# JuanLuisGonzalez/FAL_net

Hardware: AMD Instinct MI355X
Metric: stereo-pairs/sec Stage-1 step @256x512 N=49 (higher is better)
Workload: dtype bf16; 1 GPU; Stage-1 training step (BASELINE configs[1]), batch 8/GPU, 256x512, N=49, seeded weights, seeded VGG19; global_batch=8, parallelism=dp1, launch=eager launches, recorded sequences issued by falnet_replay (C)

## Files before the change

### fal_net_amd/_lib.py

```python
import ctypes as C
import os
import threading

import torch

F32, BF16, F16 = 0, 1, 2
ACT_NONE, ACT_ELU, ACT_RELU = 0, 1, 2
OUT_NHWC, OUT_PLANAR_F32 = 0, 1
CPAD = 32

DETERMINISTIC = os.environ.get("FALNET_DETERMINISTIC") == "1"

def ab(name, default):
    if os.environ.get("FALNET_AB") != "1":
        return default
    return os.environ.get(name, default)


_LIB_PATH = os.environ.get("FALNET_LIB") or os.path.join(os.path.dirname(os.path.abspath(__file__)), "libfalnet_hip.so")


class Src(C.Structure):
    _fields_ = [("ptr", C.c_void_p), ("C", C.c_int32), ("H", C.c_int32), ("W", C.c_int32),
                ("sb", C.c_int64), ("sy", C.c_int64), ("sx", C.c_int64)]
# ... 57 lines not shown
_P, _I, _L, _F, _D = C.c_void_p, C.c_int, C.c_int64, C.c_float, C.c_double
SIGNATURES = {
    "falnet_version": [],
    "falnet_last_error": [],
    "falnet_channel_pad": [_I],
    "falnet_set_device": [_I],
    "falnet_set_deterministic": [_I],
    "falnet_get_deterministic": [],
    "falnet_conv2d": [C.POINTER(Conv), _P],
    "falnet_conv3x3_c3": [_P, _P, _P, _P, _I, _I, _I, _I, _I, _I, _P],
    "falnet_conv2d_multi": [C.POINTER(Conv), _I, _P],
    "falnet_conv2d_kernel_name": [C.POINTER(Conv), C.c_char_p, _I],
    "falnet_wgrad_workspace_bytes": [C.POINTER(Wgrad)],
    "falnet_wgrad": [C.POINTER(Wgrad), _P],
    "falnet_wgrad_fuses_bias": [C.POINTER(Wgrad)],
    "falnet_wgrad_reduce": [_P, _I, _I, _I, _I, _P, _I, _I, _I, _I, _I, _P],
    "falnet_bias_grad": [_P, _L, _I, _I, _P, _I, _I, _P],
    "falnet_pack_weights_batched": [_P, _I, _I, _I, _P],
    "falnet_adam_pack_batched": [_P, _I, _I, _I, _L, _L, _L, _P, _F, _F, _F, _F, _P, _P],
    "falnet_adam_ranges": [_P, _L, _L, _L, _P, _I, _P, _F, _F, _F, _F, _P, _P],
    "falnet_adam_tick": [_P, _P, _P],
    "falnet_pack_up2_batched": [_P, _I, _I, _I, _P],
    "falnet_wgrad_reduce_batched": [_P, _I, _I, _I, _P],
    "falnet_wgrad_reduce_blocks": [_I, _I, _I],
    "falnet_bias_grad_batched": [_P, _I, _I, _I, _P],
    "falnet_bias_grad_batched_det": [_P, _I, _I, _I, _P, _L, _P],
    "falnet_pack_weights": [_P, _I, _I, _I, _I, _I, _I, _I, _P, _P, _I, _P],
    "falnet_nchw_to_nhwc": [_P, _P, _I, _I, _I, _I, _I, _I, _P],
    "falnet_nhwc_to_nchw": [_P, _P, _I, _I, _I, _I, _I, _I, _P],
    "falnet_upsample_bwd": [_P, _P, _P, _I, _I, _I, _I, _I, _I, _I, _P],
# ... 305 lines not shown
```

### fal_net_amd/csrc/conv.hip

```cpp
#include <limits.h>
#include <stdlib.h>
#include <type_traits>
#include "common.h"
#include "conv_epilogue.h"

#define CONV_THREADS 256
#define CONV_BM 128
#define ROWB 64
#define ROWP 80

template <typename T> struct KC;
template <> struct KC<float> { static constexpr int value = 16; };
template <> struct KC<bf16_t> { static constexpr int value = 32; };
template <> struct KC<f16_t> { static constexpr int value = 32; };

template <typename T> struct Vec8 {
    uint4 v;
    __device__ __forceinline__ void load(const T* p) { v = *reinterpret_cast<const uint4*>(p); }
    __device__ __forceinline__ void store(T* p) const { *reinterpret_cast<uint4*>(p) = v; }
    __device__ __forceinline__ float get(int i) const {
        const unsigned w = (&v.x)[i >> 1];
        return (i & 1) ? H16<T>::hi(w) : H16<T>::lo(w);
    }
    __device__ __forceinline__ void set8(const float (&f)[8]) {
// ... 3058 lines not shown
        const dim3 eg((unsigned)((total + 255) / 256 > 1024 ? 1024 : (total + 255) / 256), (unsigned)n);
#define SPLITK_M(T) hipLaunchKernelGGL(splitk_epilogue_multi_kernel<T>, eg, dim3(256), 0, st, pp)
        FALNET_DISPATCH_DTYPE(descs[0].dtype, SPLITK_M);
#undef SPLITK_M
    }
    FALNET_RETURN_LAUNCH();
}

static inline int round32(int v) { return (v + 31) / 32 * 32; }

extern "C" int64_t falnet_wgrad_workspace_bytes(const falnet_wgrad_t* p) {
    if (!p) return -1;
    return (int64_t)p->nsplit * p->ntaps * round32(p->gC) * p->cin_total * (int64_t)sizeof(float);
}

enum WgradKernel { WGK_BAD = -1, WGK_TAP = 0, WGK_PATCH11, WGK_PATCH12, WGK_PATCH21, WGK_S2, WGK_C3, WGK_ROWS, WGK_ROWS_S2, WGK_WAVE };
bool falnet_wgrad_rows_applicable(const falnet_wgrad_t& p);
int falnet_wgrad_rows_launch(const falnet_wgrad_t& p, hipStream_t st);
bool falnet_wgrad_rows_s2_applicable(const falnet_wgrad_t& p);
int falnet_wgrad_rows_s2_launch(const falnet_wgrad_t& p, hipStream_t st);
bool falnet_wgrad_wave_applicable(const falnet_wgrad_t& p);
int falnet_wgrad_wave_launch(const falnet_wgrad_t& p, hipStream_t st);
bool falnet_wgrad_c3wave_applicable(const falnet_wgrad_t& p);
int falnet_wgrad_c3wave_launch(const falnet_wgrad_t& p, hipStream_t st);

static bool canonical_taps9(const falnet_wgrad_t& p) {
    if (p.ntaps != 9) return false;
    for (int t = 0; t < 9; ++t)
        if (p.tap_dy[t] != t / 3 - 1 || p.tap_dx[t] != t % 3 - 1) return false;
    return true;
}

static WgradKernel choose_wgrad_kernel(const falnet_wgrad_t& p) {
    const int w_rows = round32(p.gC);
    const bool h16 = p.dtype == FALNET_BF16 || p.dtype == FALNET_F16;
    const bool canon = canonical_taps9(p);
    if (p.up2 && p.variant != 7) { falnet_set_error("wgrad: up2 (a deconv layer's gradient on the low-resolution grid) is a mode of variant 7 only"); return WGK_BAD; }
    if (p.variant == 6) {
        const bool ok = h16 && canon && p.isy == 1 && p.isx == 1 && p.TH == p.IH && p.TW == p.IW && p.gC == 32 && w_rows == 32 && p.cin_total == 32 && p.nsrc == 1;
// ... 4 lines not shown
        bool ok = h16 && canon && p.isy == 2 && p.isx == 2 && p.TW >= 16 && p.TH == (p.IH + 1) / 2 && p.TW == (p.IW + 1) / 2;
        for (int s = 0; s < p.nsrc && ok; ++s) ok = p.src[s].C % 32 == 0 && ((p.src[s].H == p.IH && p.src[s].W == p.IW) || (p.src[s].sy == 0 && p.src[s].sx == 0));
        if (!ok) { falnet_set_error("wgrad: variant 5 needs a 16-bit 3x3 stride-2 pad-1 launch with sources at the input size"); return WGK_BAD; }
        return WGK_S2;
    }
    if (p.variant == 8) {
        if (!falnet_wgrad_rows_s2_applicable(p)) { falnet_set_error("wgrad: variant 8 needs a 16-bit 3x3 stride-2 pad-1 launch with ONE source at the input size"); return WGK_BAD; }
        return WGK_ROWS_S2;
    }
    if (p.variant == 9) {
        if (!falnet_wgrad_wave_applicable(p)) { falnet_set_error("wgrad: variant 9 needs a 16-bit dense 3x3 stride-1 launch over ONE 32-channel NHWC source at the launch size, gC 32 or 64, TW >= 32"); return WGK_BAD; }
        return WGK_WAVE;
    }
    if (p.variant == 7) {
        if (!falnet_wgrad_rows_applicable(p)) { falnet_set_error("wgrad: variant 7 needs a 16-bit dense 3x3 stride-1 launch with sources at the launch size or half of it (up2: ONE source at the launch size, nsplit a multiple of 4)"); return WGK_BAD; }
        return WGK_ROWS;
    }
    const bool dense = canon && p.isy == 1 && p.isx == 1 && p.TH == p.IH && p.TW == p.IW && p.TW >= 16 && !g_disable_patch && p.variant != 1;
    if (dense) {
        if (p.variant == 3 || p.variant == 4) {
            const bool co2 = p.variant == 3;
            if (!(h16 && (co2 ? w_rows : p.cin_total) % 64 == 0)) { falnet_set_error("wgrad: variant %d needs 16-bit operands and a channel count that is a multiple of 64", p.variant); return WGK_BAD; }
            return co2 ? WGK_PATCH12 : WGK_PATCH21;
        }
        return WGK_PATCH11;
    }
    return WGK_TAP;
}

static int check_wgrad_desc(const falnet_wgrad_t& p) {
    FALNET_CHECK_ARG(p.dtype == FALNET_F32 || p.dtype == FALNET_BF16 || p.dtype == FALNET_F16, "wgrad: bad dtype %d", p.dtype);
// ... 4 lines not shown
            if (int r = check_src(p.src[s], 32, "wgrad")) return r;
            ctot += p.src[s].C;
        }
        FALNET_CHECK_ARG(ctot == p.cin_total, "wgrad: sources carry %d channels, cin_total=%d", ctot, p.cin_total);
    } else {
        FALNET_CHECK_ARG(p.src[0].ptr && p.src[0].C == 3, "wgrad: variant 6 needs a 3-channel planar f32 source");
    }
    FALNET_CHECK_ARG(p.gout && p.gC > 0 && p.gC % 32 == 0 && p.nsplit >= 1 && p.ntaps >= 1 && p.ntaps <= 9, "wgrad: bad argument");
    FALNET_CHECK_ARG(p.B > 0 && p.TH > 0 && p.TW > 0, "wgrad: empty shape");
    FALNET_CHECK_ARG(p.cout >= 0 && p.cout <= p.gC, "wgrad: cout=%d exceeds gC=%d", p.cout, p.gC);
    return 0;
}

static bool wgrad_kernel_fuses_bias(WgradKernel k) {
    if (falnet_deterministic()) return false;
    return k == WGK_PATCH11 || k == WGK_PATCH12 || k == WGK_PATCH21 || k == WGK_S2 || k == WGK_C3 || k == WGK_ROWS || k == WGK_ROWS_S2 || k == WGK_WAVE;
}

extern "C" int falnet_wgrad_fuses_bias(const falnet_wgrad_t* pp) {
    if (!pp || check_wgrad_desc(*pp) != 0) return 0;
    return wgrad_kernel_fuses_bias(choose_wgrad_kernel(*pp)) ? 1 : 0;
}

extern "C" int falnet_wgrad(const falnet_wgrad_t* pp, void* stream) {
    FALNET_ENTER(stream);
    FALNET_CHECK_ARG(pp, "wgrad: null descriptor");
    falnet_wgrad_t p = *pp;
    if (int r = check_wgrad_desc(p)) return r;
    FALNET_CHECK_ARG(p.partial, "wgrad: no workspace");
    if (p.cout == 0) p.cout = p.gC;
    const int w_rows = round32(p.gC);
    const WgradKernel k = choose_wgrad_kernel(p);
    if (k == WGK_BAD) return -1;
    if (p.bias_grad && !wgrad_kernel_fuses_bias(k)) {
        falnet_set_error("wgrad: bias_grad is set but the selected kernel (%d) cannot fuse it -- ask falnet_wgrad_fuses_bias first", (int)k);
        return -3;
    }
    hipStream_t st = (hipStream_t)stream;
    const int tiles_x = (p.TW + WP_TW - 1) / WP_TW, tiles_y = (p.TH + WP_TH - 1) / WP_TH;
    const int npatch = p.B * tiles_x * tiles_y;
    const int pps = (npatch + p.nsplit - 1) / p.nsplit;
    switch (k) {
    case WGK_ROWS:
        return falnet_wgrad_rows_launch(p, st);
    case WGK_ROWS_S2:
        return falnet_wgrad_rows_s2_launch(p, st);
    case WGK_WAVE:
        return falnet_wgrad_wave_launch(p, st);
    case WGK_C3:
        if (falnet_wgrad_c3wave_applicable(p)) return falnet_wgrad_c3wave_launch(p, st);
#define WG_C3(T) hipLaunchKernelGGL(HIP_KERNEL_NAME(wgrad3x3_c3_kernel<T>), dim3(1, 1, p.nsplit), dim3(WC3_THREADS), 0, st, p, w_rows, tiles_x, tiles_y, pps)
        FALNET_DISPATCH_16(p.dtype, WG_C3);
        break;
    case WGK_S2:
#define WG_S2_2(T) hipLaunchKernelGGL(HIP_KERNEL_NAME(wgrad3x3_s2_kernel<T, 2>), dim3(p.cin_total / 32, w_rows / 64, p.nsplit), dim3(WP_THREADS), 0, st, p, w_rows, tiles_x, tiles_y, pps)
#define WG_S2_1(T) hipLaunchKernelGGL(HIP_KERNEL_NAME(wgrad3x3_s2_kernel<T, 1>), dim3(p.cin_total / 32, w_rows / 32, p.nsplit), dim3(WP_THREADS), 0, st, p, w_rows, tiles_x, tiles_y, pps)
        if (w_rows % 64 == 0) FALNET_DISPATCH_16(p.dtype, WG_S2_2);
        else FALNET_DISPATCH_16(p.dtype, WG_S2_1);
        break;
// ... 76 lines not shown
```

### fal_net_amd/csrc/wgrad_rows.hip

```cpp
#include <stdlib.h>
#include "common.h"

typedef float f32x16 __attribute__((ext_vector_type(16)));
typedef __bf16 bf16x8 __attribute__((ext_vector_type(8)));
typedef _Float16 f16x8 __attribute__((ext_vector_type(8)));
typedef short s16x4 __attribute__((ext_vector_type(4)));
typedef short s16x8 __attribute__((ext_vector_type(8)));

template <typename T> struct Mma16;
template <> struct Mma16<bf16_t> {
    static __device__ __forceinline__ f32x16 mma(s16x8 a, s16x8 b, f32x16 c) {
        return __builtin_amdgcn_mfma_f32_32x32x16_bf16(__builtin_bit_cast(bf16x8, a), __builtin_bit_cast(bf16x8, b), c, 0, 0, 0);
    }
    static __device__ __forceinline__ float f32(short v) { return __uint_as_float(((unsigned)(unsigned short)v) << 16); }
};
template <> struct Mma16<f16_t> {
    static __device__ __forceinline__ f32x16 mma(s16x8 a, s16x8 b, f32x16 c) {
        return __builtin_amdgcn_mfma_f32_32x32x16_f16(__builtin_bit_cast(f16x8, a), __builtin_bit_cast(f16x8, b), c, 0, 0, 0);
    }
    static __device__ __forceinline__ float f32(short v) { return (float)__builtin_bit_cast(_Float16, v); }
};

#define WR_THREADS 256
#define WR_TW 32
// ... 1200 lines not shown
            float* dst = p.partial + (((int64_t)split * 9 + dy * 3 + dx) * w_rows) * p.cin_total;
#pragma unroll
            for (int j4 = 0; j4 < 4; ++j4) {
                const float4 o = *reinterpret_cast<const float4*>(red + ((dy * 3 + dx) * 4 + j4) * 256);
                const float v[4] = {acc[dy][dx][4 * j4] + o.x, acc[dy][dx][4 * j4 + 1] + o.y, acc[dy][dx][4 * j4 + 2] + o.z, acc[dy][dx][4 * j4 + 3] + o.w};
#pragma unroll
                for (int e = 0; e < 4; ++e) {
                    const int j = 4 * j4 + e;
                    const int co = co0 + 32 * c_t + (j & 3) + 8 * (j >> 2) + 4 * h;
                    if (ci < p.cin_total && co < w_rows) dst[(int64_t)co * p.cin_total + ci] = v[e];
                }
            }
        }
}

bool falnet_wgrad_rows_s2_applicable(const falnet_wgrad_t& p) {
    if (p.dtype != FALNET_BF16 && p.dtype != FALNET_F16) return false;
    if (p.ntaps != 9 || p.isy != 2 || p.isx != 2 || p.TH != (p.IH + 1) / 2 || p.TW != (p.IW + 1) / 2) return false;
    for (int t = 0; t < 9; ++t)
        if (p.tap_dy[t] != t / 3 - 1 || p.tap_dx[t] != t % 3 - 1) return false;
    if (p.gC % 32 || p.cin_total % 32 || p.nsrc != 1) return false;
    const falnet_src_t& S = p.src[0];
    if (S.C != p.cin_total || S.H != p.IH || S.W != p.IW || S.sx == 0 || S.sy == 0) return false;
    if ((int64_t)p.B * ((p.TW + WR_TW - 1) / WR_TW) * p.TH >= (1ll << 30)) return false;
    return true;
}

int falnet_wgrad_rows_s2_launch(const falnet_wgrad_t& p, hipStream_t st) {
    const int w_rows = (p.gC + 31) / 32 * 32;
    const int ntci = (p.cin_total + 63) / 64, ntco = (w_rows + 63) / 64;
// ... 68 lines not shown
    if (form == 84) {
        if (p.dtype == FALNET_F16) hipLaunchKernelGGL(HIP_KERNEL_NAME(wgrad3x3_rows8_kernel<f16_t, 4, 0, true, true, 4>), grid, dim3(WR8_THREADS), 0, st, p, w_rows, ntci, ntiles, nstrips);
        else hipLaunchKernelGGL(HIP_KERNEL_NAME(wgrad3x3_rows8_kernel<bf16_t, 4, 0, true, true, 4>), grid, dim3(WR8_THREADS), 0, st, p, w_rows, ntci, ntiles, nstrips);
        FALNET_RETURN_LAUNCH();
    }
#endif
    if (p.up2) {
        if (p.dtype == FALNET_F16) hipLaunchKernelGGL(HIP_KERNEL_NAME(wgrad3x3_rows16_kernel<f16_t, 4, 2, true>), grid, dim3(WR8_THREADS), 0, st, p, w_rows, ntci, ntiles, nstrips);
        else hipLaunchKernelGGL(HIP_KERNEL_NAME(wgrad3x3_rows16_kernel<bf16_t, 4, 2, true>), grid, dim3(WR8_THREADS), 0, st, p, w_rows, ntci, ntiles, nstrips);
        FALNET_RETURN_LAUNCH();
    }
    if (p.dtype == FALNET_F16) hipLaunchKernelGGL(HIP_KERNEL_NAME(wgrad3x3_rows16_kernel<f16_t, 4, 2, false>), grid, dim3(WR8_THREADS), 0, st, p, w_rows, ntci, ntiles, nstrips);
    else hipLaunchKernelGGL(HIP_KERNEL_NAME(wgrad3x3_rows16_kernel<bf16_t, 4, 2, false>), grid, dim3(WR8_THREADS), 0, st, p, w_rows, ntci, ntiles, nstrips);
    FALNET_RETURN_LAUNCH();
}
```

### fal_net_amd/ops.py

```python
import ctypes as C
import os
import sys

import torch

from . import _lib as L

CPAD = L.CPAD
H16 = (torch.bfloat16, torch.float16)
TYPE_SYM = {torch.bfloat16: "DF16b", torch.float16: "DF16_", torch.float32: "f"}

TIMER = None
AUTOTUNE = os.environ.get("FALNET_AUTOTUNE", "1") != "0"
DETERMINISTIC = L.DETERMINISTIC
UP2W = L.ab("FALNET_UP2W", "0") == "1"
UP2D = L.ab("FALNET_UP2D", "1") == "1"


_PKG_CACHE = os.path.join(os.path.dirname(os.path.abspath(__file__)), "autotune_cache.json")
_CACHE_PATH = os.environ.get("FALNET_AUTOTUNE_CACHE", _PKG_CACHE)
_CACHE_WRITABLE = ("FALNET_AUTOTUNE_CACHE" in os.environ and _CACHE_PATH != "0") or os.environ.get("FALNET_AUTOTUNE_CACHE_WRITE") == "1"
_GATES = {"FALNET_NO_DMA": "0", "FALNET_WS2": "1", "FALNET_S2F_DMA": "1", "FALNET_S2D_DMA": "1", "FALNET_S2_SPLITK": "1",
          "FALNET_GATHER_NARROW": "0", "FALNET_S2_MULTI": None, "FALNET_SMALL_TILE_DMA": "1", "FALNET_UP2": "1", "FALNET_DEEP": "1", "FALNET_TILE8": "1"}
if os.environ.get("FALNET_AB") == "1" and any(os.environ.get(k, v) != v for k, v in _GATES.items()):
# ... 509 lines not shown
                lib.falnet_conv2d(ref, st)
            e1.record()
            e1.synchronize()
            tt = e0.elapsed_time(e1)
            t = tt if t is None else min(t, tt)
        if _AUTOTUNE_LOG:
            print(f"[autotune] M={M} w_rows={w_rows} Cout={Cout} ntaps={d.ntaps} nsrc={d.nsrc} v{v} k{k}: {t / reps * 1e3:.1f} us", file=sys.stderr)
        if best_t is None or t < best_t:
            best, best_t = (v, k), t
    return best


def _wgrad_plan(dtype, srcs, taps, stride_in, B, TH, TW, IH, IW, cin_pad, cout_pad, max_slabs, target_wgs=1536, up2=False):
    M = B * TH * TW
    h16 = dtype in (torch.bfloat16, torch.float16)
    tn = TYPE_SYM[dtype]
    dense = len(taps) == 9 and stride_in == 1 and TW >= 16
    c3 = len(srcs) == 1 and srcs[0].C == 3
    npatch = B * ((TH + 3) // 4) * ((TW + 31) // 32)
    if c3:
        assert h16 and dense and cout_pad == 32 and cin_pad == 32, "variant 6: 16-bit first layer, Cout 32"
        variant, nsplit, sym = 6, max(1, min(_WGRAD_WGS, npatch)), f"_Z18wgrad3x3_c3_kernelI{tn}Ev14falnet_wgrad_tiiii"
        if IW % 4 == 0 and TW >= 32 and not DETERMINISTIC:
            nsplit = max(1, min(_WGRAD_WAVE_WGS, B * ((TW + 31) // 32) * TH // (8 * _WGRAD_WAVE_MIN_ROWS)))
            sym = f"_Z22wgrad3x3_c3wave_kernelI{tn}Ev14falnet_wgrad_ti"
    elif _wgrad_s2(dtype, taps, stride_in, TH, TW, IH, IW, srcs) and _wgrad_wave_s2(srcs, IH, IW, TW, cin_pad, cout_pad):
        units = B * ((TW + 31) // 32) * TH
        nsplit = max(1, min(_WGRAD_WAVE_WGS, units // _WGRAD_WAVE_MIN_ROWS))
        variant, sym = 9, f"_Z22wgrad3x3_wave32_kernelI{tn}Li2ELb1EEv14falnet_wgrad_ti"
    elif _wgrad_s2(dtype, taps, stride_in, TH, TW, IH, IW, srcs) and _wgrad_rows_s2(srcs, IH, IW, TW, cin_pad, cout_pad):
        tiles = ((cin_pad + 63) // 64) * ((cout_pad + 63) // 64)
        units = B * ((TW + 31) // 32) * TH
        nsplit = max(1, min(_WGRAD_ROWS_WGS // tiles, units // _WGRAD_ROWS_MIN_ROWS))
        if nsplit >= 8:
            nsplit -= nsplit % 8
        variant, sym = 8, f"_Z23wgrad3x3_rows8s2_kernelI{tn}Li2EEv14falnet_wgrad_tiiii"
    elif _wgrad_s2(dtype, taps, stride_in, TH, TW, IH, IW, srcs):
        tiles = (cin_pad // 32) * (cout_pad // (64 if cout_pad % 64 == 0 else 32))
        variant, nsplit = 5, max(1, min((_WGRAD_WGS + tiles - 1) // tiles, npatch))
        sym = f"_Z18wgrad3x3_s2_kernelI{tn}Li{2 if cout_pad % 64 == 0 else 1}EEv14falnet_wgrad_tiiii"
    elif _wgrad_wave(dtype, dense, srcs, IH, IW, TW, cin_pad, cout_pad) and not up2:
        npw = 8 // (cout_pad // 32)
        units = B * ((TW + 31) // 32) * TH
        nsplit = max(1, min(_WGRAD_WAVE_WGS, units // (npw * _WGRAD_WAVE_MIN_ROWS)))
        variant, sym = 9, f"_Z22wgrad3x3_wave32_kernelI{tn}Li{cout_pad // 32}ELb0EEv14falnet_wgrad_ti"
    elif _wgrad_rows(dtype, dense, srcs, IH, IW, TW, cin_pad, cout_pad):
        tiles = ((cin_pad + 63) // 64) * ((cout_pad + 63) // 64)
        units = B * ((TW + 31) // 32) * TH * (4 if up2 else 1)
        nsplit = max(1, min(_WGRAD_ROWS_WGS // tiles, units // _WGRAD_ROWS_MIN_ROWS))
        if nsplit >= 8:
            nsplit -= nsplit % 8
        if up2:
            nsplit = max(4, nsplit - nsplit % 4)
            max_slabs -= max_slabs % 4
            if max_slabs < 4:
                raise ValueError("up2 weight gradient: the slab budget holds fewer than four slabs")
        variant, sym = 7, f"_Z22wgrad3x3_rows16_kernelI{tn}Li4ELi2ELb{int(up2)}EEv14falnet_wgrad_tiiii"
    elif up2:
        raise ValueError("up2 weight gradient: the row-streaming kernel does not apply")
    elif dense:
        co2 = _wgrad_co2(dtype, dense, cin_pad, cout_pad)
        tiles = (cin_pad // 32) * (cout_pad // 32) // (2 if co2 else 1)
        nsplit = max(1, min((_WGRAD_WGS + tiles - 1) // tiles, npatch))
        variant = 3 if co2 else 0
        sym = f"_Z21wgrad3x3_patch_kernelI{tn}Li1ELi{2 if co2 else 1}EEv14falnet_wgrad_tiiii"
    else:
        tiles = ((cin_pad + 63) // 64) * ((cout_pad + 63) // 64) * len(taps)
        variant, nsplit, sym = 0, max(1, min((target_wgs + tiles - 1) // tiles, (M + 255) // 256)), f"_Z12wgrad_kernelI{tn}Ev14falnet_wgrad_ti"
    return variant, max(1, min(nsplit, max_slabs)), sym


def _fill_wgrad(d, dtype, srcs, IH, IW, gout, taps, stride_in, B, TH, TW, pc):
    d.nsrc = len(srcs)
    for i, s in enumerate(srcs):
        d.src[i] = s
    d.IH, d.IW = IH, IW
    gC = gout.shape[-1]
    d.gout, d.gC, d.cout = gout.data_ptr(), gC, pc.cout
    _fill_taps(d, taps)
    d.isy = d.isx = stride_in
    d.B, d.TH, d.TW = B, TH, TW
    d.cin_total = pc.cin_pad
    d.dtype = L.dtype_code(dtype)

# ... 4 lines not shown
    if lib.falnet_wgrad_fuses_bias(C.byref(d)) != 1:
        return False
    d.bias_grad = grad_b.data_ptr()
    return True



def wgrad_calls(dtype, srcs, IH, IW, gout, taps, stride_in, B, TH, TW, pc, grad_w, grad_b, ws, target_wgs=1536,
                name="wgrad", flops=0, up2=False):
    lib = L.lib()
    d = L.Wgrad()
    _fill_wgrad(d, dtype, srcs, IH, IW, gout, taps, stride_in, B, TH, TW, pc)
    gC = gout.shape[-1]
    M = B * TH * TW * (4 if up2 else 1)
    slab = len(taps) * pad_c(gC) * pc.cin_pad * 4
    d.variant, nsplit, sym = _wgrad_plan(dtype, srcs, taps, stride_in, B, TH, TW, IH, IW, pc.cin_pad, pad_c(gC), ws.numel() * 4 // slab,
                                         target_wgs, up2=up2)
    d.nsplit = nsplit
    d.up2 = int(up2)
    d.partial = ws.data_ptr()
    assert lib.falnet_wgrad_workspace_bytes(C.byref(d)) <= ws.numel() * 4, "wgrad workspace too small"
    ref = C.byref(d)
    c0_real, c0_pad = pc.group_channels()
    npix = M
    keep = (d, srcs, gout, grad_w, grad_b, ws)

    def k_wgrad(accumulate=0, _keep=keep):
        L.check(lib.falnet_wgrad(ref, L.stream_ptr()), name)

    fused_bias = _fuse_bias(lib, d, grad_b)

    def k_reduce(accumulate=0):
        st = L.stream_ptr()
        L.check(lib.falnet_wgrad_reduce(L.ptr(ws), d.nsplit, len(taps), pad_c(gC), pc.cin_pad, L.ptr(grad_w), pc.cout, pc.cin, c0_real, c0_pad,
# ... 72 lines not shown
    SLAB_CAP = int(L.ab("FALNET_SLAB_CAP_MB", "32")) << 20

    def __init__(self, dtype, device):
        self.dtype, self.device = dtype, device
        self.items, self.bias = [], []
        self.ws = None
        self.accumulate = 1

    def add(self, srcs, IH, IW, gout, taps, stride_in, B, TH, TW, pc, grad_w, grad_b, name="wgrad", flops=0, bucket=0, up2=False):
        lib = L.lib()
        d = L.Wgrad()
        _fill_wgrad(d, self.dtype, srcs, IH, IW, gout, taps, stride_in, B, TH, TW, pc)
        gC = gout.shape[-1]
        M = B * TH * TW * (4 if up2 else 1)
        slab = len(taps) * pad_c(gC) * pc.cin_pad * 4
        d.variant, nsplit, sym = _wgrad_plan(self.dtype, srcs, taps, stride_in, B, TH, TW, IH, IW, pc.cin_pad, pad_c(gC), max(1, self.SLAB_CAP // slab),
                                             up2=up2)
        d.nsplit = nsplit
        d.up2 = int(up2)
        ref = C.byref(d)
        keep = (d, srcs, gout, grad_w, grad_b)

        post = []

        def launch(_keep=keep):
            L.check(lib.falnet_wgrad(ref, L.stream_ptr()), name)
        c0_real, c0_pad = pc.group_channels()
        self.items.append(dict(bucket=bucket, post=post, d=d, bytes=nsplit * slab, nsplit=nsplit, ntaps=len(taps), w_rows=pad_c(gC), cin_total=pc.cin_pad,
                               cout=pc.cout, cin=pc.cin, c0_real=c0_real, c0_pad=c0_pad, grad=grad_w))
        if not _fuse_bias(lib, d, grad_b) and grad_b is not None:
            self.bias.append(dict(bucket=bucket, g=gout, npix=M, gC=gC, cout=pc.cout, db=grad_b))
        t_launch = _timed(sym, flops, 0, launch, name)

        def launch_and_reduce():
# ... 111 lines not shown
```

### include/falnet_hip.h

```cpp
#ifndef FALNET_HIP_H
#define FALNET_HIP_H

#include <stdint.h>

#ifdef __cplusplus
extern "C" {
#endif

enum { FALNET_F32 = 0, FALNET_BF16 = 1, FALNET_F16 = 2 };
enum { FALNET_ACT_NONE = 0, FALNET_ACT_ELU = 1, FALNET_ACT_RELU = 2 };
enum { FALNET_OUT_NHWC = 0, FALNET_OUT_PLANAR_F32 = 1 };

int falnet_version(void);
const char* falnet_last_error(void);
int falnet_channel_pad(int dtype);
int falnet_set_device(int device);
int falnet_set_deterministic(int on);
int falnet_get_deterministic(void);

typedef struct {
    const void* ptr;
    int32_t C;
    int32_t H, W;
    int64_t sb, sy, sx;
// ... 49 lines not shown
    int32_t gC;
    int32_t ntaps;
    int32_t tap_dy[9], tap_dx[9];
    int32_t isy, isx;
    int32_t B, TH, TW;
    int32_t cin_total;
    int32_t nsplit;
    float* partial;
    int32_t dtype;
    int32_t variant;
    float* bias_grad;
    int32_t cout;
    int32_t up2;
} falnet_wgrad_t;
int falnet_wgrad_fuses_bias(const falnet_wgrad_t* p);
int64_t falnet_wgrad_workspace_bytes(const falnet_wgrad_t* p);
int falnet_wgrad(const falnet_wgrad_t* p, void* stream);
int falnet_wgrad_reduce(const float* partial, int nsplit, int ntaps, int cout_pad, int cin_total,
                        float* grad, int cout, int cin, int c0_real, int c0_pad, int accumulate, void* stream);
int falnet_bias_grad(const void* g, int64_t npix, int gC, int cout, float* db,
                     int accumulate, int dtype, void* stream);

int falnet_wgrad_reduce_blocks(int cout, int cin_total, int groups);
typedef struct {
    const float* partial; float* grad;
    int32_t nsplit, ntaps, w_rows, cin_total, cout, cin, c0_real, c0_pad, groups, block_begin;
} falnet_reduce_t;
typedef struct {
    const void* g; float* db; int64_t npix;
    int32_t gC, cout, blocks, block_begin;
// ... 135 lines not shown
```

Before: 1530 stereo-pairs/s.

## Add rows32 wgrad kernel processing two row pairs per step for non-up2 variant 7

Adds a new weight-gradient kernel for the row-streaming 3x3 stride-1 path. It consumes two output rows per pipeline step with a double-size LDS ring slot, and splits the row range between two wave groups that reduce their results through LDS at the end. The aim is fewer barriers per row and more MFMA reuse of loaded gradient and input rows. It becomes the default for non-up2 variant 7, with an env override back to rows16. Kernel-name reporting moves from Python into a C API so profiling symbols match the new dispatch. The cost is higher LDS and register use, which may reduce occupancy.

```diff
diff --git a/fal_net_amd/_lib.py b/fal_net_amd/_lib.py
--- a/fal_net_amd/_lib.py
+++ b/fal_net_amd/_lib.py
@@ -95,6 +95,7 @@
     "falnet_wgrad_workspace_bytes": [C.POINTER(Wgrad)],
     "falnet_wgrad": [C.POINTER(Wgrad), _P],
     "falnet_wgrad_fuses_bias": [C.POINTER(Wgrad)],
+    "falnet_wgrad_kernel_name": [C.POINTER(Wgrad), C.c_char_p, _I],
     "falnet_wgrad_reduce": [_P, _I, _I, _I, _I, _P, _I, _I, _I, _I, _I, _P],
     "falnet_bias_grad": [_P, _L, _I, _I, _P, _I, _I, _P],
     "falnet_pack_weights_batched": [_P, _I, _I, _I, _P],
diff --git a/fal_net_amd/csrc/conv.hip b/fal_net_amd/csrc/conv.hip
--- a/fal_net_amd/csrc/conv.hip
+++ b/fal_net_amd/csrc/conv.hip
@@ -3096,15 +3096,21 @@
     return (int64_t)p->nsplit * p->ntaps * round32(p->gC) * p->cin_total * (int64_t)sizeof(float);
 }
 
-enum WgradKernel { WGK_BAD = -1, WGK_TAP = 0, WGK_PATCH11, WGK_PATCH12, WGK_PATCH21, WGK_S2, WGK_C3, WGK_ROWS, WGK_ROWS_S2, WGK_WAVE };
+enum WgradKernel { WGK_BAD = -1, WGK_TAP = 0, WGK_PATCH11, WGK_PATCH12, WGK_PATCH21, WGK_S2, WGK_C3, WGK_ROWS, WGK_ROWS_S2, WGK_WAVE, WGK_ROWS32 };
 bool falnet_wgrad_rows_applicable(const falnet_wgrad_t& p);
 int falnet_wgrad_rows_launch(const falnet_wgrad_t& p, hipStream_t st);
+int falnet_wgrad_rows32_launch(const falnet_wgrad_t& p, hipStream_t st);
 bool falnet_wgrad_rows_s2_applicable(const falnet_wgrad_t& p);
 int falnet_wgrad_rows_s2_launch(const falnet_wgrad_t& p, hipStream_t st);
 bool falnet_wgrad_wave_applicable(const falnet_wgrad_t& p);
 int falnet_wgrad_wave_launch(const falnet_wgrad_t& p, hipStream_t st);
 bool falnet_wgrad_c3wave_applicable(const falnet_wgrad_t& p);
 int falnet_wgrad_c3wave_launch(const falnet_wgrad_t& p, hipStream_t st);
+
+static bool wr_rows16_forced() {
+    const char* e = falnet_ab_env("FALNET_WR_ROWS16");
+    return e && e[0] == '1';
+}
 
 static bool canonical_taps9(const falnet_wgrad_t& p) {
     if (p.ntaps != 9) return false;
@@ -3139,7 +3145,7 @@
     }
     if (p.variant == 7) {
         if (!falnet_wgrad_rows_applicable(p)) { falnet_set_error("wgrad: variant 7 needs a 16-bit dense 3x3 stride-1 launch with sources at the launch size or half of it (up2: ONE source at the launch size, nsplit a multiple of 4)"); return WGK_BAD; }
-        return WGK_ROWS;
+        return p.up2 || wr_rows16_forced() ? WGK_ROWS : WGK_ROWS32;
     }
     const bool dense = canon && p.isy == 1 && p.isx == 1 && p.TH == p.IH && p.TW == p.IW && p.TW >= 16 && !g_disable_patch && p.variant != 1;
     if (dense) {
@@ -3174,12 +3180,38 @@
 
 static bool wgrad_kernel_fuses_bias(WgradKernel k) {
     if (falnet_deterministic()) return false;
-    return k == WGK_PATCH11 || k == WGK_PATCH12 || k == WGK_PATCH21 || k == WGK_S2 || k == WGK_C3 || k == WGK_ROWS || k == WGK_ROWS_S2 || k == WGK_WAVE;
+    return k == WGK_PATCH11 || k == WGK_PATCH12 || k == WGK_PATCH21 || k == WGK_S2 || k == WGK_C3 || k == WGK_ROWS || k == WGK_ROWS32 || k == WGK_ROWS_S2 || k == WGK_WAVE;
 }
 
 extern "C" int falnet_wgrad_fuses_bias(const falnet_wgrad_t* pp) {
     if (!pp || check_wgrad_desc(*pp) != 0) return 0;
     return wgrad_kernel_fuses_bias(choose_wgrad_kernel(*pp)) ? 1 : 0;
+}
+
+extern "C" int falnet_wgrad_kernel_name(const falnet_wgrad_t* pp, char* buf, int len) {
+    FALNET_CHECK_ARG(pp && buf && len > 0, "wgrad_kernel_name: bad argument");
+    if (int r = check_wgrad_desc(*pp)) return r;
+    const falnet_wgrad_t& p = *pp;
+    const WgradKernel k = choose_wgrad_kernel(p);
+    if (k == WGK_BAD) return -1;
+    const char* t = p.dtype == FALNET_BF16 ? "DF16b" : p.dtype == FALNET_F16 ? "DF16_" : "f";
+    const int w_rows = round32(p.gC);
+    switch (k) {
+    case WGK_ROWS32: snprintf(buf, len, "_Z22wgrad3x3_rows32_kernelI%sLi2ELi2EEv14falnet_wgrad_tiiii", t); break;
+    case WGK_ROWS: snprintf(buf, len, "_Z22wgrad3x3_rows16_kernelI%sLi4ELi2ELb%dEEv14falnet_wgrad_tiiii", t, p.up2 ? 1 : 0); break;
+    case WGK_ROWS_S2: snprintf(buf, len, "_Z23wgrad3x3_rows8s2_kernelI%sLi2EEv14falnet_wgrad_tiiii", t); break;
+    case WGK_WAVE: snprintf(buf, len, "_Z22wgrad3x3_wave32_kernelI%sLi%dELb%dEEv14falnet_wgrad_ti", t, p.isy == 2 || p.gC == 64 ? 2 : 1, p.isy == 2 ? 1 : 0); break;
+    case WGK_C3:
+        if (falnet_wgrad_c3wave_applicable(p)) snprintf(buf, len, "_Z22wgrad3x3_c3wave_kernelI%sEv14falnet_wgrad_ti", t);
+        else snprintf(buf, len, "_Z18wgrad3x3_c3_kernelI%sEv14falnet_wgrad_tiiii", t);
+        break;
+    case WGK_S2: snprintf(buf, len, "_Z18wgrad3x3_s2_kernelI%sLi%dEEv14falnet_wgrad_tiiii", t, w_rows % 64 == 0 ? 2 : 1); break;
+    case WGK_PATCH12: snprintf(buf, len, "_Z21wgrad3x3_patch_kernelI%sLi1ELi2EEv14falnet_wgrad_tiiii", t); break;
+    case WGK_PATCH21: snprintf(buf, len, "_Z21wgrad3x3_patch_kernelI%sLi2ELi1EEv14falnet_wgrad_tiiii", t); break;
+    case WGK_PATCH11: snprintf(buf, len, "_Z21wgrad3x3_patch_kernelI%sLi1ELi1EEv14falnet_wgrad_tiiii", t); break;
+    default: snprintf(buf, len, "_Z12wgrad_kernelI%sEv14falnet_wgrad_ti", t); break;
+    }
+    return 0;
 }
 
 extern "C" int falnet_wgrad(const falnet_wgrad_t* pp, void* stream) {
@@ -3203,6 +3235,8 @@
     switch (k) {
     case WGK_ROWS:
         return falnet_wgrad_rows_launch(p, st);
+    case WGK_ROWS32:
+        return falnet_wgrad_rows32_launch(p, st);
     case WGK_ROWS_S2:
         return falnet_wgrad_rows_s2_launch(p, st);
     case WGK_WAVE:
diff --git a/fal_net_amd/csrc/wgrad_rows.hip b/fal_net_amd/csrc/wgrad_rows.hip
--- a/fal_net_amd/csrc/wgrad_rows.hip
+++ b/fal_net_amd/csrc/wgrad_rows.hip
@@ -1238,6 +1238,315 @@
         }
 }
 
+#define WR32_SLOT (2 * WR8_SLOT)
+#ifndef WR32_D
+#define WR32_D 2
+#define WR32_SPB 2
+#endif
+
+template <int K>
+__device__ __forceinline__ void wr32_vmcnt() {
+    if constexpr (K == 12) asm volatile("s_waitcnt vmcnt(12)" ::: "memory");
+    else if constexpr (K == 10) asm volatile("s_waitcnt vmcnt(10)" ::: "memory");
+    else wr_vmcnt<K>();
+}
+
+template <typename T, int D, int SPB>
+__global__ __launch_bounds__(WR8_THREADS, 2) void wgrad3x3_rows32_kernel(const falnet_wgrad_t p, int w_rows, int ntci, int ntiles, int nstrips) {
+    constexpr int NS = D + SPB;
+    static_assert(D >= 1 && D <= 3 && (SPB == 1 || SPB == 2) && D >= SPB && D - SPB <= 2, "prefetch distance / steps per barrier");
+    constexpr int LDS_BYTES = NS * WR32_SLOT > WR8_RED ? NS * WR32_SLOT : WR8_RED;
+    static_assert(LDS_BYTES <= 160 * 1024, "ring + reduction space must fit in LDS");
+    __shared__ __attribute__((aligned(1024))) char lds[LDS_BYTES];
+    const int tid = threadIdx.x, lane = tid & 63;
+    const int wave = __builtin_amdgcn_readfirstlane(tid >> 6);
+    const unsigned lds_base = (unsigned)(unsigned long)(wr_lptr_t)lds;
+    const int nsplit = p.nsplit;
+    int tile, split;
+    {
+        const int wg = blockIdx.x;
+        if ((nsplit & 7) == 0) {
+            const int idx = wg >> 3;
+            split = (idx / ntiles) * 8 + (wg & 7);
+            tile = idx % ntiles;
+        } else {
+            tile = wg % ntiles;
+            split = wg / ntiles;
+        }
+    }
+    const int ci0 = (tile % ntci) * 64, co0 = (tile / ntci) * 64;
+    const int grp = wave >> 2, pw = wave & 3;
+    const int c_t = wave & 1, a_t = (wave >> 1) & 1;
+    const int H = p.TH, TW = p.TW, gC = p.gC, IH = p.IH;
+    const int R = p.B * nstrips * H;
+    const int u0 = (int)((int64_t)R * split / nsplit), u1 = (int)((int64_t)R * (split + 1) / nsplit);
+    const int um = u0 + ((u1 - u0 + 1) >> 1);
+    const int gu0 = grp ? um : u0, gu1 = grp ? u1 : um;
+
+    const int pl = lane >> 3, cpos = lane & 7;
+    const int gch = cpos ^ ((((pl >> 1) & 1) << 2) | ((pw & 1) << 1));
+    const char* const zero_page = reinterpret_cast<const char*>(g_wr_zero);
+    const bool g_chok = co0 + 8 * gch < gC;
+    const int ch = ci0 + 8 * gch;
+    const bool x_chok = ch < p.cin_total;
+    const int c_first = p.src[0].C;
+    const bool second = p.nsrc > 1 && ch >= c_first;
+    const falnet_src_t& S = second ? p.src[1] : p.src[0];
+    const int l_hs = S.H != IH ? 1 : 0, l_ws = S.W != p.IW ? 1 : 0;
+    const int64_t l_sy = S.sy, l_sx = S.sx, l_sb = S.sb;
+    const T* const l_ptr = reinterpret_cast<const T*>(S.ptr) + (second ? ch - c_first : ch);
+
+    auto load_item = [&](Wr8Item& c, int u) {
+        c.u = u;
+        const int bs = u / H;
+        c.y0 = u - bs * H;
+        c.n = min((bs + 1) * H, gu1) - u;
+        c.T = (c.n + 3) >> 1;
+        c.b = bs / nstrips;
+        c.x0 = (bs - c.b * nstrips) * WR_TW;
+        c.t = 0;
+    };
+    auto count_steps = [&](int a, int e1) {
+        int n = 0;
+        for (int u = a; u < e1;) {
+            const int e = min((u / H + 1) * H, e1);
+            n += (e - u + 3) >> 1;
+            u = e;
+        }
+        return n;
+    };
+    const int nst_g = count_steps(gu0, gu1);
+    const int nst = max(nst_g, count_steps(grp ? u0 : um, grp ? um : u1));
+
+    const char* gptr = zero_page;
+    const char* xptr = zero_page;
+    const char* x4ptr = zero_page;
+    unsigned g_inc = 0, x_inc = 0, x4_inc = 0, x_r1 = 0, x4_r1 = 0;
+    auto item_pointers = [&](const Wr8Item& c) {
+        const int gx = c.x0 + 8 * pw + pl;
+        const bool g_ok = g_chok && gx < TW;
+        const int xa = c.x0 - 1 + 8 * pw + pl;
+        const bool x_ok = x_chok && xa >= 0 && xa < p.IW;
+        const int xb = c.x0 - 1 + 32 + pl;
+        const bool x4_ok = x_chok && pl < 2 && xb < p.IW;
+        const unsigned xi = (unsigned)((l_hs ? l_sy : 2 * l_sy) * (int)sizeof(T));
+        g_inc = g_ok ? (unsigned)(2 * TW * gC * (int)sizeof(T)) : 0u;
+        x_inc = x_ok ? xi : 0u;
+        x4_inc = x4_ok ? xi : 0u;
+        gptr = g_ok ? reinterpret_cast<const char*>(reinterpret_cast<const T*>(p.gout) + (((int64_t)c.b * H + c.y0) * TW + gx) * gC + co0 + 8 * gch) : zero_page;
+        const int i = c.y0 - 1;
+        const int64_t rowoff = (int64_t)c.b * l_sb + (int64_t)(i >> l_hs) * l_sy;
+        xptr = x_ok ? reinterpret_cast<const char*>(l_ptr + rowoff + (int64_t)(xa >> l_ws) * l_sx) : zero_page;
+        x4ptr = x4_ok ? reinterpret_cast<const char*>(l_ptr + rowoff + (int64_t)(xb >> l_ws) * l_sx) : zero_page;
+        const unsigned r1 = (unsigned)((((i + 1) >> l_hs) - (i >> l_hs)) * l_sy * (int)sizeof(T));
+        x_r1 = x_ok ? r1 : 0u;
+        x4_r1 = x4_ok ? r1 : 0u;
+    };
+    auto issue_piece = [&](const Wr8Item& c, int slot, int k) {
+        const unsigned base = lds_base + slot * WR32_SLOT + grp * WR8_SLOT;
+        const int rs = k & 1;
+        if (k < 2) {
+            const bool gv = 2 * c.t + rs < c.n;
+            wr_glds16(gv ? gptr + (rs ? g_inc >> 1 : 0u) : zero_page, base + rs * WR_GROW + pw * 1024);
+            if (rs) gptr += g_inc;
+            return;
+        }
+        const int i = c.y0 - 1 + 2 * c.t + rs;
+        const bool xv = i >= 0 && i < IH;
+        if (k < 4) {
+            wr_glds16(xv ? xptr + (rs ? x_r1 : 0u) : zero_page, base + 2 * WR_GROW + rs * WR_XROW + pw * 1024);
+            if (rs) xptr += x_inc;
+        } else if (pw == 2 * rs) {
+            wr_glds16(xv ? x4ptr + (rs ? x4_r1 : 0u) : zero_page, base + 2 * WR_GROW + rs * WR_XROW + 4 * 1024);
+            x4ptr += x4_inc;
+        }
+    };
+
+    const int i16 = lane & 15, g16 = lane >> 4;
+    const int q = i16 >> 2, pc = i16 & 3;
+    auto frag_off = [&](int cb16, int pshift, int second_read) {
+        const int px = 8 * g16 + q + pshift + 4 * second_read;
+        const int chunk = 2 * cb16 + (pc >> 1);
+        const int sw = (((px >> 1) & 1) << 2) | (((px >> 3) & 1) << 1);
+        return px * 128 + ((chunk ^ sw) * 16) + (pc & 1) * 8;
+    };
+    int offA[2], offB[3][2];
+#pragma unroll
+    for (int rd = 0; rd < 2; ++rd) {
+        offA[rd] = grp * WR8_SLOT + frag_off(2 * c_t, 0, rd);
+#pragma unroll
+        for (int dx = 0; dx < 3; ++dx) offB[dx][rd] = grp * WR8_SLOT + 2 * WR_GROW + frag_off(2 * a_t, dx, rd);
+    }
+    auto frag = [&](const char* base, const int (&off)[2], int odd) -> s16x8 {
+        const s16x4 v0 = __builtin_amdgcn_ds_read_tr16_b64_v4i16((wr_lds_v4)(base + (off[0] ^ (odd << 5))));
+        const s16x4 v1 = __builtin_amdgcn_ds_read_tr16_b64_v4i16((wr_lds_v4)(base + (off[1] ^ (odd << 5))));
+        return __builtin_shufflevector(v0, v1, 0, 1, 2, 3, 4, 5, 6, 7);
+    };
+
+    f32x4_t acc[3][3][2][2];
+#pragma unroll
+    for (int dy = 0; dy < 3; ++dy)
+#pragma unroll
+        for (int dx = 0; dx < 3; ++dx)
+#pragma unroll
+            for (int cc = 0; cc < 2; ++cc)
+#pragma unroll
+                for (int ca = 0; ca < 2; ++ca) acc[dy][dx][cc][ca] = f32x4_t{0.f, 0.f, 0.f, 0.f};
+    s16x8 w_a[2], w_b[2];
+#pragma unroll
+    for (int cc = 0; cc < 2; ++cc)
+#pragma unroll
+        for (int j = 0; j < 8; ++j) w_a[cc][j] = w_b[cc][j] = 0;
+    const bool a_live = ci0 + 32 * a_t < p.cin_total && co0 + 32 * c_t < gC;
+    const bool do_bias = p.bias_grad != nullptr && (tile % ntci) == 0 && a_t == 0;
+    float bsum[2] = {0.f, 0.f};
+
+    Wr8Item ci_, cc_;
+    if (nst_g > 0) {
+        load_item(ci_, gu0);
+        cc_ = ci_;
+        item_pointers(ci_);
+#pragma unroll
+        for (int d = 0; d < D; ++d) {
+            if (d < nst_g) {
+#pragma unroll
+                for (int k = 0; k < 6; ++k) issue_piece(ci_, d, k);
+                if (d + 1 < nst_g && ++ci_.t == ci_.T) {
+                    load_item(ci_, ci_.u + ci_.n);
+                    item_pointers(ci_);
+                }
+            }
+        }
+    }
+    int slot = 0, islot = D;
+    for (int g = 0; g < nst; ++g) {
+        const bool do_issue = g + D < nst_g;
+        if (SPB == 1 || (g & (SPB - 1)) == 0) {
+            const int k = max(0, min(D - SPB, nst_g - g - SPB));
+            if ((pw & 1) == 0) {
+                if (k >= 2) wr32_vmcnt<(D - SPB >= 2 ? 10 : 0)>();
+                else if (k == 1) wr32_vmcnt<(D - SPB >= 1 ? 5 : 0)>();
+                else wr32_vmcnt<0>();
+            } else {
+                if (k >= 2) wr32_vmcnt<(D - SPB >= 2 ? 8 : 0)>();
+                else if (k == 1) wr32_vmcnt<(D - SPB >= 1 ? 4 : 0)>();
+                else wr32_vmcnt<0>();
+            }
+            asm volatile("s_waitcnt lgkmcnt(0)" ::: "memory");
+            __builtin_amdgcn_s_barrier();
+        }
+        auto piece = [&](int kk) {
+            if (do_issue) {
+                __builtin_amdgcn_sched_barrier(0);
+                issue_piece(ci_, islot, kk);
+                __builtin_amdgcn_sched_barrier(0);
+            }
+        };
+        if (g < nst_g) {
+            const char* sb = lds + slot * WR32_SLOT;
+            const int t2 = 2 * cc_.t, n = cc_.n;
+            const int i0 = cc_.y0 - 1 + t2;
+            const bool vx0 = a_live && i0 >= 0 && i0 < IH, vx1 = a_live && i0 + 1 >= 0 && i0 + 1 < IH;
+            auto vr = [&](int r) { return (unsigned)r < (unsigned)n; };
+            auto mm = [&](int dy, const s16x8 (&A)[2], const s16x8 (&X)[3][2]) {
+#pragma unroll
+                for (int dx = 0; dx < 3; ++dx)
+#pragma unroll
+                    for (int cc = 0; cc < 2; ++cc)
+#pragma unroll
+                        for (int ca = 0; ca < 2; ++ca) acc[dy][dx][cc][ca] = H16<T>::mma16(A[cc], X[dx][ca], acc[dy][dx][cc][ca]);
+            };
+            s16x8 n_a[2], n_b[2], xr[3][2];
+#pragma unroll
+            for (int cc = 0; cc < 2; ++cc) n_a[cc] = frag(sb, offA, cc);
+#pragma unroll
+            for (int dx = 0; dx < 3; ++dx)
+#pragma unroll
+                for (int ca = 0; ca < 2; ++ca) xr[dx][ca] = frag(sb, offB[dx], ca);
+            if (vx0 && vr(t2)) mm(0, n_a, xr);
+            piece(0);
+            if (vx0 && vr(t2 - 1)) mm(1, w_b, xr);
+            piece(2);
+            if (vx0 && vr(t2 - 2)) mm(2, w_a, xr);
+            piece(4);
+#pragma unroll
+            for (int cc = 0; cc < 2; ++cc) n_b[cc] = frag(sb + WR_GROW, offA, cc);
+#pragma unroll
+            for (int dx = 0; dx < 3; ++dx)
+#pragma unroll
+                for (int ca = 0; ca < 2; ++ca) xr[dx][ca] = frag(sb + WR_XROW, offB[dx], ca);
+            if (vx1 && vr(t2 + 1)) mm(0, n_b, xr);
+            piece(1);
+            if (vx1 && vr(t2)) mm(1, n_a, xr);
+            piece(3);
+            if (vx1 && vr(t2 - 1)) mm(2, w_b, xr);
+            piece(5);
+            if (do_bias) {
+#pragma unroll
+                for (int cc = 0; cc < 2; ++cc)
+#pragma unroll
+                    for (int j = 0; j < 8; ++j) bsum[cc] += Mma16<T>::f32(n_a[cc][j]) + Mma16<T>::f32(n_b[cc][j]);
+            }
+#pragma unroll
+            for (int cc = 0; cc < 2; ++cc) {
+                w_a[cc] = n_a[cc];
+                w_b[cc] = n_b[cc];
+            }
+            if (g + 1 < nst_g && ++cc_.t == cc_.T) load_item(cc_, cc_.u + cc_.n);
+            if (do_issue && g + D + 1 < nst_g && ++ci_.t == ci_.T) {
+                load_item(ci_, ci_.u + ci_.n);
+                item_pointers(ci_);
+            }
+        }
+        slot = slot + 1 == NS ? 0 : slot + 1;
+        islot = islot + 1 == NS ? 0 : islot + 1;
+    }
+
+    asm volatile("s_waitcnt vmcnt(0) lgkmcnt(0)" ::: "memory");
+    __builtin_amdgcn_s_barrier();
+    float* red = reinterpret_cast<float*>(lds) + (wave & 3) * (36 * 256) + lane * 4;
+    if (grp == 1) {
+#pragma unroll
+        for (int dy = 0; dy < 3; ++dy)
+#pragma unroll
+            for (int dx = 0; dx < 3; ++dx)
+#pragma unroll
+                for (int cc = 0; cc < 2; ++cc)
+#pragma unroll
+                    for (int ca = 0; ca < 2; ++ca) *reinterpret_cast<f32x4_t*>(red + (((dy * 3 + dx) * 2 + cc) * 2 + ca) * 256) = acc[dy][dx][cc][ca];
+    }
+    __syncthreads();
+    if (do_bias) {
+#pragma unroll
+        for (int cc = 0; cc < 2; ++cc) {
+            float b = bsum[cc];
+            b += __shfl_xor(b, 16, 64);
+            b += __shfl_xor(b, 32, 64);
+            const int co = co0 + 32 * c_t + 16 * cc + i16;
+            if (g16 == 0 && co < p.cout) atomicAdd(p.bias_grad + co, b);
+        }
+    }
+    if (grp == 1) return;
+#pragma unroll
+    for (int dy = 0; dy < 3; ++dy)
+#pragma unroll
+        for (int dx = 0; dx < 3; ++dx) {
+            float* dst = p.partial + (((int64_t)split * 9 + dy * 3 + dx) * w_rows) * p.cin_total;
+#pragma unroll
+            for (int cc = 0; cc < 2; ++cc)
+#pragma unroll
+                for (int ca = 0; ca < 2; ++ca) {
+                    const f32x4_t o = *reinterpret_cast<const f32x4_t*>(red + (((dy * 3 + dx) * 2 + cc) * 2 + ca) * 256);
+                    const int ci = ci0 + 32 * a_t + 16 * ca + i16;
+#pragma unroll
+                    for (int f = 0; f < 4; ++f) {
+                        const int co = co0 + 32 * c_t + 16 * cc + 4 * g16 + f;
+                        if (ci < p.cin_total && co < w_rows) dst[(int64_t)co * p.cin_total + ci] = acc[dy][dx][cc][ca][f] + o[f];
+                    }
+                }
+        }
+}
+
 bool falnet_wgrad_rows_s2_applicable(const falnet_wgrad_t& p) {
     if (p.dtype != FALNET_BF16 && p.dtype != FALNET_F16) return false;
     if (p.ntaps != 9 || p.isy != 2 || p.isx != 2 || p.TH != (p.IH + 1) / 2 || p.TW != (p.IW + 1) / 2) return false;
@@ -1336,3 +1645,18 @@
     else hipLaunchKernelGGL(HIP_KERNEL_NAME(wgrad3x3_rows16_kernel<bf16_t, 4, 2, false>), grid, dim3(WR8_THREADS), 0, st, p, w_rows, ntci, ntiles, nstrips);
     FALNET_RETURN_LAUNCH();
 }
+
+int falnet_wgrad_rows32_launch(const falnet_wgrad_t& p, hipStream_t st) {
+    if (p.up2) {
+        falnet_set_error("wgrad rows32: up2 runs on the rows16 kernel");
+        return -1;
+    }
+    const int w_rows = (p.gC + 31) / 32 * 32;
+    const int ntci = (p.cin_total + 63) / 64, ntco = (w_rows + 63) / 64;
+    const int ntiles = ntci * ntco;
+    const int nstrips = (p.TW + WR_TW - 1) / WR_TW;
+    const dim3 grid((unsigned)(ntiles * p.nsplit));
+    if (p.dtype == FALNET_F16) hipLaunchKernelGGL(HIP_KERNEL_NAME(wgrad3x3_rows32_kernel<f16_t, WR32_D, WR32_SPB>), grid, dim3(WR8_THREADS), 0, st, p, w_rows, ntci, ntiles, nstrips);
+    else hipLaunchKernelGGL(HIP_KERNEL_NAME(wgrad3x3_rows32_kernel<bf16_t, WR32_D, WR32_SPB>), grid, dim3(WR8_THREADS), 0, st, p, w_rows, ntci, ntiles, nstrips);
+    FALNET_RETURN_LAUNCH();
+}
diff --git a/fal_net_amd/ops.py b/fal_net_amd/ops.py
--- a/fal_net_amd/ops.py
+++ b/fal_net_amd/ops.py
@@ -547,36 +547,33 @@
 def _wgrad_plan(dtype, srcs, taps, stride_in, B, TH, TW, IH, IW, cin_pad, cout_pad, max_slabs, target_wgs=1536, up2=False):
     M = B * TH * TW
     h16 = dtype in (torch.bfloat16, torch.float16)
-    tn = TYPE_SYM[dtype]
     dense = len(taps) == 9 and stride_in == 1 and TW >= 16
     c3 = len(srcs) == 1 and srcs[0].C == 3
     npatch = B * ((TH + 3) // 4) * ((TW + 31) // 32)
     if c3:
         assert h16 and dense and cout_pad == 32 and cin_pad == 32, "variant 6: 16-bit first layer, Cout 32"
-        variant, nsplit, sym = 6, max(1, min(_WGRAD_WGS, npatch)), f"_Z18wgrad3x3_c3_kernelI{tn}Ev14falnet_wgrad_tiiii"
+        variant, nsplit = 6, max(1, min(_WGRAD_WGS, npatch))
         if IW % 4 == 0 and TW >= 32 and not DETERMINISTIC:
             nsplit = max(1, min(_WGRAD_WAVE_WGS, B * ((TW + 31) // 32) * TH // (8 * _WGRAD_WAVE_MIN_ROWS)))
-            sym = f"_Z22wgrad3x3_c3wave_kernelI{tn}Ev14falnet_wgrad_ti"
     elif _wgrad_s2(dtype, taps, stride_in, TH, TW, IH, IW, srcs) and _wgrad_wave_s2(srcs, IH, IW, TW, cin_pad, cout_pad):
         units = B * ((TW + 31) // 32) * TH
         nsplit = max(1, min(_WGRAD_WAVE_WGS, units // _WGRAD_WAVE_MIN_ROWS))
-        variant, sym = 9, f"_Z22wgrad3x3_wave32_kernelI{tn}Li2ELb1EEv14falnet_wgrad_ti"
+        variant = 9
     elif _wgrad_s2(dtype, taps, stride_in, TH, TW, IH, IW, srcs) and _wgrad_rows_s2(srcs, IH, IW, TW, cin_pad, cout_pad):
         tiles = ((cin_pad + 63) // 64) * ((cout_pad + 63) // 64)
         units = B * ((TW + 31) // 32) * TH
         nsplit = max(1, min(_WGRAD_ROWS_WGS // tiles, units // _WGRAD_ROWS_MIN_ROWS))
         if nsplit >= 8:
             nsplit -= nsplit % 8
-        variant, sym = 8, f"_Z23wgrad3x3_rows8s2_kernelI{tn}Li2EEv14falnet_wgrad_tiiii"
+        variant = 8
     elif _wgrad_s2(dtype, taps, stride_in, TH, TW, IH, IW, srcs):
         tiles = (cin_pad // 32) * (cout_pad // (64 if cout_pad % 64 == 0 else 32))
         variant, nsplit = 5, max(1, min((_WGRAD_WGS + tiles - 1) // tiles, npatch))
-        sym = f"_Z18wgrad3x3_s2_kernelI{tn}Li{2 if cout_pad % 64 == 0 else 1}EEv14falnet_wgrad_tiiii"
     elif _wgrad_wave(dtype, dense, srcs, IH, IW, TW, cin_pad, cout_pad) and not up2:
         npw = 8 // (cout_pad // 32)
         units = B * ((TW + 31) // 32) * TH
         nsplit = max(1, min(_WGRAD_WAVE_WGS, units // (npw * _WGRAD_WAVE_MIN_ROWS)))
-        variant, sym = 9, f"_Z22wgrad3x3_wave32_kernelI{tn}Li{cout_pad // 32}ELb0EEv14falnet_wgrad_ti"
+        variant = 9
     elif _wgrad_rows(dtype, dense, srcs, IH, IW, TW, cin_pad, cout_pad):
         tiles = ((cin_pad + 63) // 64) * ((cout_pad + 63) // 64)
         units = B * ((TW + 31) // 32) * TH * (4 if up2 else 1)
@@ -588,7 +585,7 @@
             max_slabs -= max_slabs % 4
             if max_slabs < 4:
                 raise ValueError("up2 weight gradient: the slab budget holds fewer than four slabs")
-        variant, sym = 7, f"_Z22wgrad3x3_rows16_kernelI{tn}Li4ELi2ELb{int(up2)}EEv14falnet_wgrad_tiiii"
+        variant = 7
     elif up2:
         raise ValueError("up2 weight gradient: the row-streaming kernel does not apply")
     elif dense:
@@ -596,11 +593,16 @@
         tiles = (cin_pad // 32) * (cout_pad // 32) // (2 if co2 else 1)
         nsplit = max(1, min((_WGRAD_WGS + tiles - 1) // tiles, npatch))
         variant = 3 if co2 else 0
-        sym = f"_Z21wgrad3x3_patch_kernelI{tn}Li1ELi{2 if co2 else 1}EEv14falnet_wgrad_tiiii"
     else:
         tiles = ((cin_pad + 63) // 64) * ((cout_pad + 63) // 64) * len(taps)
-        variant, nsplit, sym = 0, max(1, min((target_wgs + tiles - 1) // tiles, (M + 255) // 256)), f"_Z12wgrad_kernelI{tn}Ev14falnet_wgrad_ti"
-    return variant, max(1, min(nsplit, max_slabs)), sym
+        variant, nsplit = 0, max(1, min((target_wgs + tiles - 1) // tiles, (M + 255) // 256))
+    return variant, max(1, min(nsplit, max_slabs))
+
+
+def _wgrad_kernel_name(lib, d):
+    buf = C.create_string_buffer(160)
+    L.check(lib.falnet_wgrad_kernel_name(C.byref(d), buf, 160), "wgrad_kernel_name")
+    return buf.value.decode()
 
 
 def _fill_wgrad(d, dtype, srcs, IH, IW, gout, taps, stride_in, B, TH, TW, pc):
@@ -635,10 +637,11 @@
     gC = gout.shape[-1]
     M = B * TH * TW * (4 if up2 else 1)
     slab = len(taps) * pad_c(gC) * pc.cin_pad * 4
-    d.variant, nsplit, sym = _wgrad_plan(dtype, srcs, taps, stride_in, B, TH, TW, IH, IW, pc.cin_pad, pad_c(gC), ws.numel() * 4 // slab,
-                                         target_wgs, up2=up2)
+    d.variant, nsplit = _wgrad_plan(dtype, srcs, taps, stride_in, B, TH, TW, IH, IW, pc.cin_pad, pad_c(gC), ws.numel() * 4 // slab,
+                                    target_wgs, up2=up2)
     d.nsplit = nsplit
     d.up2 = int(up2)
+    sym = _wgrad_kernel_name(lib, d)
     d.partial = ws.data_ptr()
     assert lib.falnet_wgrad_workspace_bytes(C.byref(d)) <= ws.numel() * 4, "wgrad workspace too small"
     ref = C.byref(d)
@@ -741,10 +744,11 @@
         gC = gout.shape[-1]
         M = B * TH * TW * (4 if up2 else 1)
         slab = len(taps) * pad_c(gC) * pc.cin_pad * 4
-        d.variant, nsplit, sym = _wgrad_plan(self.dtype, srcs, taps, stride_in, B, TH, TW, IH, IW, pc.cin_pad, pad_c(gC), max(1, self.SLAB_CAP // slab),
-                                             up2=up2)
+        d.variant, nsplit = _wgrad_plan(self.dtype, srcs, taps, stride_in, B, TH, TW, IH, IW, pc.cin_pad, pad_c(gC), max(1, self.SLAB_CAP // slab),
+                                        up2=up2)
         d.nsplit = nsplit
         d.up2 = int(up2)
+        sym = _wgrad_kernel_name(lib, d)
         ref = C.byref(d)
         keep = (d, srcs, gout, grad_w, grad_b)
 
diff --git a/include/falnet_hip.h b/include/falnet_hip.h
--- a/include/falnet_hip.h
+++ b/include/falnet_hip.h
@@ -87,6 +87,7 @@
     int32_t up2;
 } falnet_wgrad_t;
 int falnet_wgrad_fuses_bias(const falnet_wgrad_t* p);
+int falnet_wgrad_kernel_name(const falnet_wgrad_t* p, char* buf, int len);
 int64_t falnet_wgrad_workspace_bytes(const falnet_wgrad_t* p);
 int falnet_wgrad(const falnet_wgrad_t* p, void* stream);
 int falnet_wgrad_reduce(const float* partial, int nsplit, int ntaps, int cout_pad, int cin_total,
```

After: 1546 stereo-pairs/s (median of 6 runs). No clear change (+1.0%).
